# Dhia-naouali/dinov3-jax

Measured on NVIDIA H100. Metric: global_crops_per_sec, higher is better.
Workload: dtype bf16

## Files before the change

dinov3-jax_b200/csrc/attention.cu:

```cuda
#include "ptx.cuh"
#include <climits>
#include <cstdlib>
#include "d3_internal.h"

namespace d3 {

constexpr float LOG2E = 1.4426950408889634f;

__device__ long long* g_attn_dbg = nullptr;
__device__ __forceinline__ void dbg_mark(int slot) {
  if (g_attn_dbg && blockIdx.x == 0 && blockIdx.y == 0 && blockIdx.z == 0 && (threadIdx.x == 0 || threadIdx.x == 200))
    g_attn_dbg[slot * 2 + (threadIdx.x == 0 ? 0 : 1)] = clock64();
}

struct AttnShape {
  int G;
  int span;
  int n_crops;
  int N;
  int nkb;
  int D;
  int H;
  float scale;
  const float* sin_t;
  const float* cos_t;
  int prefix;
};

__device__ __forceinline__ uint32_t sw128_offset(int row, int col) {
  return (uint32_t)(row * 128 + ((((col >> 3) ^ (row & 7)) & 7) << 4) + (col & 7) * 2);
}

struct RowInfo { int g, klo, khi; bool ok; };
__device__ __forceinline__ RowInfo row_info(const AttnShape& sh, int c, int q) {
  RowInfo ri;
  ri.g = min(q / sh.N, sh.G - 1);
  ri.klo = ri.g * sh.N;
  ri.khi = ri.klo + sh.N;
  ri.ok = (q < sh.span) && (c * sh.G + ri.g < sh.n_crops);
  return ri;
}

template <int NI>
__device__ __forceinline__ void online_softmax(float (&s)[4 * NI], float (&o)[32], float (&m)[2], float (&l)[2],
                                               const RowInfo (&ri)[2], int k0, int c2, float cs) {
  const int kb0 = k0 + c2;
  const bool full = k0 >= max(ri[0].klo, ri[1].klo) && k0 + 8 * NI <= min(ri[0].khi, ri[1].khi);
  float mx[2] = {-3.0e38f, -3.0e38f};
#pragma unroll
  for (int i = 0; i < NI; ++i)
#pragma unroll
    for (int j = 0; j < 4; ++j) {
      const int hh = j >> 1, kk = kb0 + 8 * i + (j & 1);
      if (full || (kk >= ri[hh].klo && kk < ri[hh].khi)) mx[hh] = fmaxf(mx[hh], s[4 * i + j]);
    }
  float corr[2], ms[2];
#pragma unroll
  for (int hh = 0; hh < 2; ++hh) {
    mx[hh] = fmaxf(mx[hh], __shfl_xor_sync(0xffffffffu, mx[hh], 1));
    mx[hh] = fmaxf(mx[hh], __shfl_xor_sync(0xffffffffu, mx[hh], 2));
    const float mn = fmaxf(m[hh], mx[hh]);
    corr[hh] = ex2_approx((m[hh] - mn) * cs);
    m[hh] = mn;
    ms[hh] = mn * cs;
    l[hh] *= corr[hh];
  }
#pragma unroll
  for (int i = 0; i < NI; ++i)
#pragma unroll
    for (int j = 0; j < 4; ++j) {
      const int hh = j >> 1, kk = kb0 + 8 * i + (j & 1);
      const float p = (full || (kk >= ri[hh].klo && kk < ri[hh].khi)) ? ex2_approx(fmaf(s[4 * i + j], cs, -ms[hh])) : 0.f;
      s[4 * i + j] = p;
      l[hh] += p;
      if (i < 8) o[4 * i + j] *= corr[hh];
    }
}

__device__ __forceinline__ void store_o_lse(const float (&o)[32], float (&l)[2], const float (&m)[2], const RowInfo (&ri)[2],
                                            const AttnShape& sh, int c, int h, int row_base, int wq0, int r_in, int c2,
                                            __nv_bfloat16* O, float* LSE) {
#pragma unroll
  for (int hh = 0; hh < 2; ++hh) {
    l[hh] += __shfl_xor_sync(0xffffffffu, l[hh], 1);
    l[hh] += __shfl_xor_sync(0xffffffffu, l[hh], 2);
    const int q = wq0 + r_in + 8 * hh;
    if (!ri[hh].ok) continue;
    const float inv = 1.f / l[hh];
    __nv_bfloat16* dst = O + (size_t)(row_base + q) * sh.D + h * 64 + c2;
#pragma unroll
    for (int i = 0; i < 8; ++i)
      *reinterpret_cast<uint32_t*>(dst + 8 * i) = pack_bf16(o[4 * i + 2 * hh] * inv, o[4 * i + 2 * hh + 1] * inv);
    if (LSE && c2 == 0)
      LSE[((size_t)(c * sh.G + ri[hh].g) * sh.H + h) * sh.N + (q - ri[hh].klo)] = m[hh] * sh.scale + logf(l[hh]);
  }
}

__global__ void __launch_bounds__(256)
attn_fwd_kernel(const __grid_constant__ CUtensorMap tmQ, const __grid_constant__ CUtensorMap tmKV,
                __nv_bfloat16* __restrict__ O, float* __restrict__ LSE, const AttnShape sh) {
  extern __shared__ uint8_t smem_raw[];
  uint8_t* smem = reinterpret_cast<uint8_t*>((reinterpret_cast<uintptr_t>(smem_raw) + 1023) & ~uintptr_t(1023));
  uint8_t* sQ = smem;
  uint8_t* sK = smem + 16384;
  uint8_t* sV = sK + sh.nkb * 8192;
  uint64_t* bar = reinterpret_cast<uint64_t*>(sV + sh.nkb * 8192);

  const int wg = threadIdx.x >> 7, t = threadIdx.x & 127;
  const int qt = blockIdx.x, h = blockIdx.y, c = blockIdx.z;
  const int q0 = qt * 128;
  const int row_base = c * sh.span;
  dbg_mark(0);
  if (threadIdx.x == 0) {
    tma_prefetch_desc(&tmQ);
    tma_prefetch_desc(&tmKV);
    mbar_init(bar, 1);
    fence_mbar_init();
  }
  __syncthreads();
  if (threadIdx.x < 32 && elect_one()) {
    mbar_expect_tx(bar, 16384 + 2 * sh.nkb * 8192);
    tma_load_2d(&tmQ, bar, sQ, h * 64, row_base + q0);
    for (int b = 0; b < sh.nkb; ++b) {
      tma_load_2d(&tmKV, bar, sK + b * 8192, sh.D + h * 64, row_base + b * 64);
      tma_load_2d(&tmKV, bar, sV + b * 8192, 2 * sh.D + h * 64, row_base + b * 64);
    }
  }
  const int wq0 = q0 + wg * 64;
  if (wq0 >= sh.span) return;
  mbar_wait(bar, 0);

  const int r_in = 16 * (t >> 5) + ((t & 31) >> 2), c2 = 2 * (t & 3);
  RowInfo ri[2];
  ri[0] = row_info(sh, c, wq0 + r_in);
  ri[1] = row_info(sh, c, wq0 + r_in + 8);
  const int b_lo = (min(wq0 / sh.N, sh.G - 1) * sh.N) >> 6;
  const int b_hi = min(sh.nkb, ((min(min(wq0 + 63, sh.span - 1) / sh.N, sh.G - 1) + 1) * sh.N + 63) >> 6);
  const float cs = sh.scale * LOG2E;
  float m[2] = {-3.0e38f, -3.0e38f}, l[2] = {0.f, 0.f};
  float o[32];
#pragma unroll
  for (int i = 0; i < 32; ++i) o[i] = 0.f;
  const uint64_t qd = gmma_desc_sw128(smem_u32(sQ + wg * 8192), 16, 1024);

#pragma unroll 1
  for (int b = b_lo; b < b_hi; ++b) {
    float s[32];
    const uint64_t kd = gmma_desc_sw128(smem_u32(sK + b * 8192), 16, 1024);
    fence_regs(o);
    wgmma_fence();
#pragma unroll
    for (int k = 0; k < 4; ++k) wgmma_m64n64k16_ss<0, 0>(s, qd + 2 * k, kd + 2 * k, k > 0 ? 1u : 0u);
    wgmma_commit();
    wgmma_wait<0>();
    fence_regs(s);
    online_softmax<8>(s, o, m, l, ri, b * 64, c2, cs);
    uint32_t a[4][4];
#pragma unroll
    for (int kk = 0; kk < 4; ++kk)
#pragma unroll
      for (int e = 0; e < 4; ++e) a[kk][e] = pack_bf16(s[8 * kk + 2 * e], s[8 * kk + 2 * e + 1]);
    const uint64_t vd = gmma_desc_sw128(smem_u32(sV + b * 8192), 8192, 1024);
    fence_regs(o);
    wgmma_fence();
#pragma unroll
    for (int kk = 0; kk < 4; ++kk) wgmma_m64n64k16_rs<1>(o, a[kk], vd + 128 * kk, 1u);
    wgmma_commit();
    wgmma_wait<0>();
    fence_regs(o);
  }
  store_o_lse(o, l, m, ri, sh, c, h, row_base, wq0, r_in, c2, O, LSE);
  dbg_mark(1);
}

constexpr int FWD_STAGES = 4, DKDV_STAGES = 3, DQ_STAGES = 4;
constexpr int RING_THREADS = 384;

__global__ void __launch_bounds__(RING_THREADS, 1)
attn_fwd_stream_kernel(const __grid_constant__ CUtensorMap tmQKV, __nv_bfloat16* __restrict__ O, float* __restrict__ LSE,
                       const AttnShape sh) {
  extern __shared__ uint8_t smem_raw[];
  uint8_t* smem = reinterpret_cast<uint8_t*>((reinterpret_cast<uintptr_t>(smem_raw) + 1023) & ~uintptr_t(1023));
  uint8_t* sQ = smem;
  uint8_t* ring = smem + 16384;
  uint64_t* full = reinterpret_cast<uint64_t*>(ring + FWD_STAGES * 32768);
  uint64_t* empty = full + FWD_STAGES;
  uint64_t* bar_q = empty + FWD_STAGES;

  const int wg = threadIdx.x >> 7, t = threadIdx.x & 127;
  const int qt = blockIdx.x, h = blockIdx.y, c = blockIdx.z;
  const int q0 = qt * 128, row_base = c * sh.N, nkb = (sh.N + 127) >> 7;
  const int n_wg = (q0 + 64 < sh.N) ? 2 : 1;
  if (threadIdx.x == 0) {
    tma_prefetch_desc(&tmQKV);
    for (int st = 0; st < FWD_STAGES; ++st) {
      mbar_init(full + st, 1);
      mbar_init(empty + st, 4 * n_wg);
    }
    mbar_init(bar_q, 1);
    fence_mbar_init();
  }
  __syncthreads();
  if (wg == 2) {
    setmaxnreg_dec<40>();
    if (threadIdx.x < 288 && elect_one()) {
      mbar_expect_tx(bar_q, 16384);
      tma_load_2d(&tmQKV, bar_q, sQ, h * 64, row_base + q0);
      for (int b = 0; b < nkb; ++b) {
        const int st = b % FWD_STAGES, u = b / FWD_STAGES;
        if (u > 0) mbar_wait(empty + st, (u - 1) & 1);
        mbar_expect_tx(full + st, 32768);
        tma_load_2d(&tmQKV, full + st, ring + st * 32768, sh.D + h * 64, row_base + b * 128);
        tma_load_2d(&tmQKV, full + st, ring + st * 32768 + 16384, 2 * sh.D + h * 64, row_base + b * 128);
      }
    }
    return;
  }
  setmaxnreg_inc<232>();
  const int wq0 = q0 + wg * 64;
  if (wq0 >= sh.N) return;
  mbar_wait(bar_q, 0);

  const int r_in = 16 * (t >> 5) + ((t & 31) >> 2), c2 = 2 * (t & 3);
  RowInfo ri[2];
  ri[0] = row_info(sh, c, wq0 + r_in);
  ri[1] = row_info(sh, c, wq0 + r_in + 8);
  const float cs = sh.scale * LOG2E;
  float m[2] = {-3.0e38f, -3.0e38f}, l[2] = {0.f, 0.f};
  float o[32];
#pragma unroll
  for (int i = 0; i < 32; ++i) o[i] = 0.f;
  const uint64_t qd = gmma_desc_sw128(smem_u32(sQ + wg * 8192), 16, 1024);

#pragma unroll 1
  for (int b = 0; b < nkb; ++b) {
    const int st = b % FWD_STAGES;
    uint8_t* sK = ring + st * 32768;
    mbar_wait(full + st, (b / FWD_STAGES) & 1);
    float s[64];
    const uint64_t kd = gmma_desc_sw128(smem_u32(sK), 16, 1024);
    fence_regs(o);
    wgmma_fence();
#pragma unroll
    for (int k = 0; k < 4; ++k) wgmma_m64n128k16_ss<0, 0>(s, qd + 2 * k, kd + 2 * k, k > 0 ? 1u : 0u);
    wgmma_commit();
    wgmma_wait<0>();
    fence_regs(s);
    online_softmax<16>(s, o, m, l, ri, b * 128, c2, cs);
    uint32_t a[8][4];
#pragma unroll
    for (int kk = 0; kk < 8; ++kk)
#pragma unroll
      for (int e = 0; e < 4; ++e) a[kk][e] = pack_bf16(s[8 * kk + 2 * e], s[8 * kk + 2 * e + 1]);
    const uint64_t vd = gmma_desc_sw128(smem_u32(sK + 16384), 8192, 1024);
    fence_regs(o);
    wgmma_fence();
#pragma unroll
    for (int kk = 0; kk < 8; ++kk) wgmma_m64n64k16_rs<1>(o, a[kk], vd + 128 * kk, 1u);
    wgmma_commit();
    wgmma_wait<0>();
    fence_regs(o);
    if (lane_id() == 0) mbar_arrive(empty + st);
  }
  store_o_lse(o, l, m, ri, sh, c, h, row_base, wq0, r_in, c2, O, LSE);
}

__global__ void attn_delta_kernel(const __nv_bfloat16* __restrict__ O, const __nv_bfloat16* __restrict__ dO,
                                  float* __restrict__ delta, long T, int N, int D, int H) {
  const long g = blockIdx.x * (long)blockDim.x + threadIdx.x;
  const int per_row = D >> 3;
  const bool ok = g < T * per_row;
  float s = 0.f;
  long row = 0;
  int c8 = 0;
  if (ok) {
    row = g / per_row;
    c8 = (int)(g % per_row);
    const uint4 a = *reinterpret_cast<const uint4*>(O + row * D + c8 * 8);
    const uint4 b = *reinterpret_cast<const uint4*>(dO + row * D + c8 * 8);
    const float2 a0 = unpack_bf16(a.x), a1 = unpack_bf16(a.y), a2 = unpack_bf16(a.z), a3 = unpack_bf16(a.w);
    const float2 b0 = unpack_bf16(b.x), b1 = unpack_bf16(b.y), b2 = unpack_bf16(b.z), b3 = unpack_bf16(b.w);
    s = a0.x * b0.x + a0.y * b0.y + a1.x * b1.x + a1.y * b1.y + a2.x * b2.x + a2.y * b2.y + a3.x * b3.x + a3.y * b3.y;
  }
  s += __shfl_xor_sync(0xffffffffu, s, 4);
  s += __shfl_xor_sync(0xffffffffu, s, 2);
  s += __shfl_xor_sync(0xffffffffu, s, 1);
  if (ok && (c8 & 7) == 0) delta[((row / N) * H + (c8 >> 3)) * N + (row % N)] = s;
}

__device__ __forceinline__ void store_grad_rows(float (&a)[32], const AttnShape& sh, int c, int row_base, int tile_row0,
                                                int r_in, int c2, int h, int third, bool rope, __nv_bfloat16* dQKV) {
#pragma unroll
  for (int hh = 0; hh < 2; ++hh) {
    const int row = tile_row0 + r_in + 8 * hh;
    const RowInfo ri = row_info(sh, c, row);
    if (!ri.ok) continue;
    const int tok = row - ri.klo;
    float v[16];
#pragma unroll
    for (int i = 0; i < 8; ++i) { v[2 * i] = a[4 * i + 2 * hh]; v[2 * i + 1] = a[4 * i + 2 * hh + 1]; }
    if (rope && sh.sin_t && tok >= sh.prefix) {
      const float* sn = sh.sin_t + (size_t)(tok - sh.prefix) * 64;
      const float* cn = sh.cos_t + (size_t)(tok - sh.prefix) * 64;
#pragma unroll
      for (int i = 0; i < 4; ++i)
#pragma unroll
        for (int j = 0; j < 2; ++j) {
          const int d = 8 * i + c2 + j;
          const float lo = v[2 * i + j], hi = v[2 * (i + 4) + j];
          v[2 * i + j] = lo * cn[d] + hi * sn[d];
          v[2 * (i + 4) + j] = hi * cn[d] - lo * sn[d];
        }
    }
    __nv_bfloat16* dst = dQKV + (size_t)(row_base + row) * (3 * sh.D) + third * sh.D + h * 64 + c2;
#pragma unroll
    for (int i = 0; i < 8; ++i) *reinterpret_cast<uint32_t*>(dst + 8 * i) = pack_bf16(v[2 * i], v[2 * i + 1]);
  }
}

__device__ __forceinline__ void p_ds_tile(const AttnShape& sh, const float* __restrict__ LSE, const float* __restrict__ Delta,
                                          int c, int h, int q0, int kt, const uint8_t* sQw, const uint8_t* sDOw,
                                          const uint8_t* sK, const uint8_t* sV, int r_in, int c2, float (&s)[64],
                                          float (&dp)[64]) {
  const float cs = sh.scale * LOG2E;
  const uint64_t qd = gmma_desc_sw128(smem_u32(sQw), 16, 1024);
  const uint64_t dod = gmma_desc_sw128(smem_u32(sDOw), 16, 1024);
  const uint64_t kd = gmma_desc_sw128(smem_u32(sK), 16, 1024);
  const uint64_t vd = gmma_desc_sw128(smem_u32(sV), 16, 1024);
  wgmma_fence();
#pragma unroll
  for (int k = 0; k < 4; ++k) {
    wgmma_m64n128k16_ss<0, 0>(s, qd + 2 * k, kd + 2 * k, k > 0 ? 1u : 0u);
    wgmma_m64n128k16_ss<0, 0>(dp, dod + 2 * k, vd + 2 * k, k > 0 ? 1u : 0u);
  }
  wgmma_commit();
  wgmma_wait<0>();
  fence_regs(s);
  fence_regs(dp);
#pragma unroll
  for (int hh = 0; hh < 2; ++hh) {
    const int q = q0 + r_in + 8 * hh;
    const RowInfo ri = row_info(sh, c, q);
    const size_t stat = ((size_t)(c * sh.G + ri.g) * sh.H + h) * sh.N + (ri.ok ? q - ri.klo : 0);
    const float lse2 = ri.ok ? LSE[stat] * LOG2E : 0.f;
    const float dl = ri.ok ? Delta[stat] : 0.f;
    const int lo = ri.ok ? ri.klo - kt * 128 : 0, hi = ri.ok ? ri.khi - kt * 128 : 0;
#pragma unroll
    for (int i = 0; i < 16; ++i)
#pragma unroll
      for (int j = 0; j < 2; ++j) {
        const int e = 4 * i + 2 * hh + j, col = 8 * i + c2 + j;
        const bool ok = col >= lo && col < hi;
        const float p = ok ? ex2_approx(fmaf(s[e], cs, -lse2)) : 0.f;
        dp[e] = ok ? (p * sh.scale) * (dp[e] - dl) : 0.f;
        s[e] = p;
      }
  }
}

__device__ __forceinline__ void stash_p_ds(const float (&s)[64], const float (&dp)[64], uint8_t* sP, uint8_t* sDS, int row,
                                           int c2) {
#pragma unroll
  for (int hh = 0; hh < 2; ++hh) {
#pragma unroll
    for (int i = 0; i < 16; ++i) {
      const uint32_t off = (i >> 3) * 16384 + sw128_offset(row + 8 * hh, (8 * i + c2) & 63);
      *reinterpret_cast<uint32_t*>(sP + off) = pack_bf16(s[4 * i + 2 * hh], s[4 * i + 2 * hh + 1]);
      *reinterpret_cast<uint32_t*>(sDS + off) = pack_bf16(dp[4 * i + 2 * hh], dp[4 * i + 2 * hh + 1]);
    }
  }
}

__device__ __forceinline__ void dkdv_mma(float (&dk)[32], float (&dv)[32], const uint8_t* sP, const uint8_t* sDS,
                                         const uint8_t* sDOt, const uint8_t* sQt, int wg) {
  const uint64_t pd = gmma_desc_sw128(smem_u32(sP + wg * 16384), 16384, 1024);
  const uint64_t sd = gmma_desc_sw128(smem_u32(sDS + wg * 16384), 16384, 1024);
  const uint64_t dod = gmma_desc_sw128(smem_u32(sDOt), 8192, 1024);
  const uint64_t qd = gmma_desc_sw128(smem_u32(sQt), 8192, 1024);
  fence_regs(dk);
  fence_regs(dv);
  wgmma_fence();
#pragma unroll
  for (int k = 0; k < 8; ++k) {
    wgmma_m64n64k16_ss<1, 1>(dv, pd + 128 * k, dod + 128 * k, 1u);
    wgmma_m64n64k16_ss<1, 1>(dk, sd + 128 * k, qd + 128 * k, 1u);
  }
  wgmma_commit();
  wgmma_wait<0>();
  fence_regs(dk);
  fence_regs(dv);
}

__device__ __forceinline__ void dq_mma(float (&dq)[32], const float (&dp)[64], const uint8_t* sK) {
  uint32_t a[8][4];
#pragma unroll
  for (int kk = 0; kk < 8; ++kk)
#pragma unroll
    for (int e = 0; e < 4; ++e) a[kk][e] = pack_bf16(dp[8 * kk + 2 * e], dp[8 * kk + 2 * e + 1]);
  const uint64_t kd = gmma_desc_sw128(smem_u32(sK), 8192, 1024);
  fence_regs(dq);
  wgmma_fence();
#pragma unroll
  for (int kk = 0; kk < 8; ++kk) wgmma_m64n64k16_rs<1>(dq, a[kk], kd + 128 * kk, 1u);
  wgmma_commit();
  wgmma_wait<0>();
  fence_regs(dq);
}

__global__ void __launch_bounds__(256)
attn_bwd_kernel(const __grid_constant__ CUtensorMap tmQKV, const __grid_constant__ CUtensorMap tmDO,
                const float* __restrict__ LSE, const float* __restrict__ Delta, __nv_bfloat16* __restrict__ dQKV,
                const AttnShape sh) {
  extern __shared__ uint8_t smem_raw[];
  uint8_t* smem = reinterpret_cast<uint8_t*>((reinterpret_cast<uintptr_t>(smem_raw) + 1023) & ~uintptr_t(1023));
  const int nQ = (sh.span + 127) / 128, nK = nQ;
  uint8_t* sQ = smem;
  uint8_t* sDO = sQ + nQ * 16384;
  uint8_t* sK = sDO + nQ * 16384;
  uint8_t* sV = sK + 16384;
  uint8_t* sP = sV + 16384;
  uint8_t* sDS = sP + 32768;
  uint64_t* bars = reinterpret_cast<uint64_t*>(sDS + 32768);
  uint64_t* bar_q = bars;
  uint64_t* bar_kv = bars + 1;

  const int wg = threadIdx.x >> 7, t = threadIdx.x & 127;
  const int r_in = 16 * (t >> 5) + ((t & 31) >> 2), c2 = 2 * (t & 3);
  const int h = blockIdx.x, c = blockIdx.y;
  const int row_base = c * sh.span;
  dbg_mark(0);
  if (threadIdx.x == 0) {
    tma_prefetch_desc(&tmQKV);
    tma_prefetch_desc(&tmDO);
    mbar_init(bar_q, 1);
    mbar_init(bar_kv, 1);
    fence_mbar_init();
  }
  __syncthreads();
  if (threadIdx.x < 32 && elect_one()) {
    mbar_expect_tx(bar_q, nQ * 2 * 16384);
    for (int qt = 0; qt < nQ; ++qt) {
      tma_load_2d(&tmQKV, bar_q, sQ + qt * 16384, h * 64, row_base + qt * 128);
      tma_load_2d(&tmDO, bar_q, sDO + qt * 16384, h * 64, row_base + qt * 128);
    }
  }
  uint32_t kv_phase = 0;
  int kv_loaded = -1;
  auto load_kv = [&](int kt) {
    if (kv_loaded == kt) return;
    __syncthreads();
    if (threadIdx.x < 32 && elect_one()) {
      mbar_expect_tx(bar_kv, 2 * 16384);
      tma_load_2d(&tmQKV, bar_kv, sK, sh.D + h * 64, row_base + kt * 128);
      tma_load_2d(&tmQKV, bar_kv, sV, 2 * sh.D + h * 64, row_base + kt * 128);
    }
    mbar_wait(bar_kv, kv_phase);
    kv_phase ^= 1;
    kv_loaded = kt;
  };
  auto p_ds = [&](int qt, int kt, float (&s)[64], float (&dp)[64]) {
    p_ds_tile(sh, LSE, Delta, c, h, qt * 128 + wg * 64, kt, sQ + qt * 16384 + wg * 8192, sDO + qt * 16384 + wg * 8192,
              sK, sV, r_in, c2, s, dp);
  };

  mbar_wait(bar_q, 0);
#pragma unroll 1
  for (int kt = 0; kt < nK; ++kt) {
    load_kv(kt);
    float dk[32], dv[32];
#pragma unroll
    for (int i = 0; i < 32; ++i) { dk[i] = 0.f; dv[i] = 0.f; }
#pragma unroll 1
    for (int qt = 0; qt < nQ; ++qt) {
      float s[64], dp[64];
      p_ds(qt, kt, s, dp);
      stash_p_ds(s, dp, sP, sDS, wg * 64 + r_in, c2);
      fence_proxy_async_smem();
      __syncthreads();
      dkdv_mma(dk, dv, sP, sDS, sDO + qt * 16384, sQ + qt * 16384, wg);
      __syncthreads();
    }
    store_grad_rows(dk, sh, c, row_base, kt * 128 + wg * 64, r_in, c2, h, 1, true, dQKV);
    store_grad_rows(dv, sh, c, row_base, kt * 128 + wg * 64, r_in, c2, h, 2, false, dQKV);
  }
#pragma unroll 1
  for (int qt = 0; qt < nQ; ++qt) {
    float dq[32];
#pragma unroll
    for (int i = 0; i < 32; ++i) dq[i] = 0.f;
#pragma unroll 1
    for (int j = 0; j < nK; ++j) {
      const int kt = (qt & 1) ? j : nK - 1 - j;
      load_kv(kt);
      float s[64], dp[64];
      p_ds(qt, kt, s, dp);
      dq_mma(dq, dp, sK);
    }
    store_grad_rows(dq, sh, c, row_base, qt * 128 + wg * 64, r_in, c2, h, 0, true, dQKV);
  }
  dbg_mark(1);
}

__global__ void __launch_bounds__(RING_THREADS, 1)
attn_bwd_dkdv_kernel(const __grid_constant__ CUtensorMap tmQKV, const __grid_constant__ CUtensorMap tmDO,
                     const float* __restrict__ LSE, const float* __restrict__ Delta, __nv_bfloat16* __restrict__ dQKV,
                     const AttnShape sh) {
  extern __shared__ uint8_t smem_raw[];
  uint8_t* smem = reinterpret_cast<uint8_t*>((reinterpret_cast<uintptr_t>(smem_raw) + 1023) & ~uintptr_t(1023));
  uint8_t* sK = smem;
  uint8_t* sV = sK + 16384;
  uint8_t* sP = sV + 16384;
  uint8_t* sDS = sP + 32768;
  uint8_t* ring = sDS + 32768;
  uint64_t* full = reinterpret_cast<uint64_t*>(ring + DKDV_STAGES * 32768);
  uint64_t* empty = full + DKDV_STAGES;
  uint64_t* bar_kv = empty + DKDV_STAGES;

  const int wg = threadIdx.x >> 7, t = threadIdx.x & 127;
  const int r_in = 16 * (t >> 5) + ((t & 31) >> 2), c2 = 2 * (t & 3);
  const int kt = blockIdx.x, h = blockIdx.y, c = blockIdx.z;
  const int row_base = c * sh.N, nq = (sh.N + 127) >> 7;
  if (threadIdx.x == 0) {
    tma_prefetch_desc(&tmQKV);
    tma_prefetch_desc(&tmDO);
    for (int st = 0; st < DKDV_STAGES; ++st) {
      mbar_init(full + st, 1);
      mbar_init(empty + st, 8);
    }
    mbar_init(bar_kv, 1);
    fence_mbar_init();
  }
  __syncthreads();
  if (wg == 2) {
    setmaxnreg_dec<40>();
    if (threadIdx.x < 288 && elect_one()) {
      mbar_expect_tx(bar_kv, 32768);
      tma_load_2d(&tmQKV, bar_kv, sK, sh.D + h * 64, row_base + kt * 128);
      tma_load_2d(&tmQKV, bar_kv, sV, 2 * sh.D + h * 64, row_base + kt * 128);
      for (int qt = 0; qt < nq; ++qt) {
        const int st = qt % DKDV_STAGES, u = qt / DKDV_STAGES;
        if (u > 0) mbar_wait(empty + st, (u - 1) & 1);
        mbar_expect_tx(full + st, 32768);
        tma_load_2d(&tmQKV, full + st, ring + st * 32768, h * 64, row_base + qt * 128);
        tma_load_2d(&tmDO, full + st, ring + st * 32768 + 16384, h * 64, row_base + qt * 128);
      }
    }
    return;
  }
  setmaxnreg_inc<232>();
  mbar_wait(bar_kv, 0);
  float dk[32], dv[32];
#pragma unroll
  for (int i = 0; i < 32; ++i) { dk[i] = 0.f; dv[i] = 0.f; }
#pragma unroll 1
  for (int qt = 0; qt < nq; ++qt) {
    const int st = qt % DKDV_STAGES;
    const uint8_t* sQt = ring + st * 32768;
    const uint8_t* sDOt = sQt + 16384;
    mbar_wait(full + st, (qt / DKDV_STAGES) & 1);
    float s[64], dp[64];
    p_ds_tile(sh, LSE, Delta, c, h, qt * 128 + wg * 64, kt, sQt + wg * 8192, sDOt + wg * 8192, sK, sV, r_in, c2, s, dp);
    stash_p_ds(s, dp, sP, sDS, wg * 64 + r_in, c2);
    fence_proxy_async_smem();
    named_bar_sync(1, 256);
    dkdv_mma(dk, dv, sP, sDS, sDOt, sQt, wg);
    if (lane_id() == 0) mbar_arrive(empty + st);
    named_bar_sync(1, 256);
  }
  store_grad_rows(dk, sh, c, row_base, kt * 128 + wg * 64, r_in, c2, h, 1, true, dQKV);
  store_grad_rows(dv, sh, c, row_base, kt * 128 + wg * 64, r_in, c2, h, 2, false, dQKV);
}

__global__ void __launch_bounds__(RING_THREADS, 1)
attn_bwd_dq_kernel(const __grid_constant__ CUtensorMap tmQKV, const __grid_constant__ CUtensorMap tmDO,
                   const float* __restrict__ LSE, const float* __restrict__ Delta, __nv_bfloat16* __restrict__ dQKV,
                   const AttnShape sh) {
  extern __shared__ uint8_t smem_raw[];
  uint8_t* smem = reinterpret_cast<uint8_t*>((reinterpret_cast<uintptr_t>(smem_raw) + 1023) & ~uintptr_t(1023));
  uint8_t* sQ = smem;
  uint8_t* sDO = sQ + 16384;
  uint8_t* ring = sDO + 16384;
  uint64_t* full = reinterpret_cast<uint64_t*>(ring + DQ_STAGES * 32768);
  uint64_t* empty = full + DQ_STAGES;
  uint64_t* bar_q = empty + DQ_STAGES;

  const int wg = threadIdx.x >> 7, t = threadIdx.x & 127;
  const int r_in = 16 * (t >> 5) + ((t & 31) >> 2), c2 = 2 * (t & 3);
  const int qt = blockIdx.x, h = blockIdx.y, c = blockIdx.z;
  const int q0 = qt * 128, row_base = c * sh.N, nk = (sh.N + 127) >> 7;
  const int n_wg = (q0 + 64 < sh.N) ? 2 : 1;
  if (threadIdx.x == 0) {
    tma_prefetch_desc(&tmQKV);
    tma_prefetch_desc(&tmDO);
    for (int st = 0; st < DQ_STAGES; ++st) {
      mbar_init(full + st, 1);
      mbar_init(empty + st, 4 * n_wg);
    }
    mbar_init(bar_q, 1);
    fence_mbar_init();
  }
  __syncthreads();
  if (wg == 2) {
    setmaxnreg_dec<40>();
    if (threadIdx.x < 288 && elect_one()) {
      mbar_expect_tx(bar_q, 32768);
      tma_load_2d(&tmQKV, bar_q, sQ, h * 64, row_base + q0);
      tma_load_2d(&tmDO, bar_q, sDO, h * 64, row_base + q0);
      for (int kt = 0; kt < nk; ++kt) {
        const int st = kt % DQ_STAGES, u = kt / DQ_STAGES;
        if (u > 0) mbar_wait(empty + st, (u - 1) & 1);
        mbar_expect_tx(full + st, 32768);
        tma_load_2d(&tmQKV, full + st, ring + st * 32768, sh.D + h * 64, row_base + kt * 128);
        tma_load_2d(&tmQKV, full + st, ring + st * 32768 + 16384, 2 * sh.D + h * 64, row_base + kt * 128);
      }
    }
    return;
  }
  setmaxnreg_inc<232>();
  const int wq0 = q0 + wg * 64;
  if (wq0 >= sh.N) return;
  mbar_wait(bar_q, 0);
  float dq[32];
#pragma unroll
  for (int i = 0; i < 32; ++i) dq[i] = 0.f;
#pragma unroll 1
  for (int kt = 0; kt < nk; ++kt) {
    const int st = kt % DQ_STAGES;
    const uint8_t* sK = ring + st * 32768;
    mbar_wait(full + st, (kt / DQ_STAGES) & 1);
    float s[64], dp[64];
    p_ds_tile(sh, LSE, Delta, c, h, wq0, kt, sQ + wg * 8192, sDO + wg * 8192, sK, sK + 16384, r_in, c2, s, dp);
    dq_mma(dq, dp, sK);
    if (lane_id() == 0) mbar_arrive(empty + st);
  }
  store_grad_rows(dq, sh, c, row_base, wq0, r_in, c2, h, 0, true, dQKV);
}

static int make_map(CUtensorMap* map, const void* ptr, long rows, int cols, int ld, int box_rows) {
  cuuint64_t dims[2] = {(cuuint64_t)cols, (cuuint64_t)rows};
  cuuint64_t strides[1] = {(cuuint64_t)ld * 2};
  cuuint32_t box[2] = {64, (cuuint32_t)box_rows};
  cuuint32_t estr[2] = {1, 1};
  return encode_tensor_map_2d_bf16(map, ptr, dims, strides, box, estr);
}

constexpr int ATTN_MAX_TOKENS = 32768;
constexpr int ATTN_FWD_RESIDENT_SPAN = 448;
constexpr int ATTN_BWD_RESIDENT_N = 384;

static int attn_shape(AttnShape* s, int n_crops, int N, int D, int H) {
  if (D != H * 64) return set_error(D3_ERR_ARG, "attention: head_dim must be 64");
  if (N <= 0 || n_crops <= 0) return set_error(D3_ERR_ARG, "attention: empty problem");
  if (N > ATTN_MAX_TOKENS) return set_error(D3_ERR_ARG, "attention: N > 32768 tokens per crop");
  if ((long)n_crops * N > INT_MAX) return set_error(D3_ERR_ARG, "attention: n_crops * N must be below 2^31 token rows");
  s->N = N; s->D = D; s->H = H; s->scale = 0.125f; s->n_crops = n_crops;
  s->sin_t = nullptr; s->cos_t = nullptr; s->prefix = 0;
  s->G = (N <= 64) ? (128 / N) : 1;
  if (s->G > n_crops) s->G = n_crops;
  s->span = s->G * N;
  s->nkb = (s->span + 63) / 64;
  return D3_OK;
}

static int stream_grid(const AttnShape& s, dim3* grid) {
  if (s.H > 65535 || s.n_crops > 65535) return set_error(D3_ERR_ARG, "attention: H and n_crops must be <= 65535 for long crops");
  *grid = dim3((s.N + 127) / 128, s.H, s.n_crops);
  return D3_OK;
}

}

using namespace d3;

extern "C" {

int d3_debug_attn_trace(long long* buf ) {
  cudaError_t e = cudaMemcpyToSymbol(g_attn_dbg, &buf, sizeof(buf));
  return e == cudaSuccess ? D3_OK : set_error(D3_ERR_CUDA, cudaGetErrorString(e));
}

int d3_attn_fwd(const void* qkv, void* o, float* lse, int n_crops, int N, int D, int H, void* stream) {
  AttnShape s;
  int rc = attn_shape(&s, n_crops, N, D, H);
  if (rc) return rc;
  const long T = (long)n_crops * N;
  if (s.span > ATTN_FWD_RESIDENT_SPAN) {
    dim3 grid;
    if ((rc = stream_grid(s, &grid))) return rc;
    CUtensorMap tqkv;
    if ((rc = make_map(&tqkv, qkv, T, 3 * D, 3 * D, 128))) return rc;
    const int smem = 16384 + FWD_STAGES * 32768 + (2 * FWD_STAGES + 1) * 8 + 1024;
    static bool cfg_stream = false;
    if (!cfg_stream) {
      cudaFuncSetAttribute(attn_fwd_stream_kernel, cudaFuncAttributeMaxDynamicSharedMemorySize, smem);
      cfg_stream = true;
    }
    attn_fwd_stream_kernel<<<grid, RING_THREADS, smem, reinterpret_cast<cudaStream_t>(stream)>>>(tqkv, (__nv_bfloat16*)o,
                                                                                                 lse, s);
    D3_CHECK_LAUNCH();
    return D3_OK;
  }
  CUtensorMap tq, tkv;
  if ((rc = make_map(&tq, qkv, T, 3 * D, 3 * D, 128))) return rc;
  if ((rc = make_map(&tkv, qkv, T, 3 * D, 3 * D, 64))) return rc;
  const int smem = 16384 + 2 * s.nkb * 8192 + 64 + 1024;
  static bool cfg = false;
  if (!cfg) { cudaFuncSetAttribute(attn_fwd_kernel, cudaFuncAttributeMaxDynamicSharedMemorySize, 200 * 1024); cfg = true; }
  dim3 grid((s.span + 127) / 128, H, (n_crops + s.G - 1) / s.G);
  attn_fwd_kernel<<<grid, 256, smem, reinterpret_cast<cudaStream_t>(stream)>>>(tq, tkv, (__nv_bfloat16*)o, lse, s);
  D3_CHECK_LAUNCH();
  return D3_OK;
}

int d3_attn_bwd(const void* qkv, const void* o, const void* d_o, const float* lse, float* delta_scratch, void* dqkv,
                int n_crops, int N, int D, int H, const float* rope_sin, const float* rope_cos, int rope_prefix,
                void* stream) {
  AttnShape s;
  int rc = attn_shape(&s, n_crops, N, D, H);
  if (rc) return rc;
  if ((rope_sin == nullptr) != (rope_cos == nullptr)) return set_error(D3_ERR_ARG, "d3_attn_bwd: sin/cos tables");
  if (!delta_scratch) return set_error(D3_ERR_ARG, "d3_attn_bwd: delta scratch buffer");
  const bool streamed = N > ATTN_BWD_RESIDENT_N;
  dim3 sgrid;
  if (streamed && (rc = stream_grid(s, &sgrid))) return rc;
  s.sin_t = rope_sin; s.cos_t = rope_cos; s.prefix = rope_prefix;
  const long T = (long)n_crops * N;
  cudaStream_t st = reinterpret_cast<cudaStream_t>(stream);
  const long threads = T * (D / 8);
  attn_delta_kernel<<<(int)((threads + 255) / 256), 256, 0, st>>>((const __nv_bfloat16*)o, (const __nv_bfloat16*)d_o,
                                                                delta_scratch, T, N, D, H);
  D3_CHECK_LAUNCH();
  CUtensorMap tqkv, tdo;
  if ((rc = make_map(&tqkv, qkv, T, 3 * D, 3 * D, 128))) return rc;
  if ((rc = make_map(&tdo, d_o, T, D, D, 128))) return rc;
  if (streamed) {
    const int smem_kv = 16384 * 2 + 32768 * 2 + DKDV_STAGES * 32768 + (2 * DKDV_STAGES + 1) * 8 + 1024;
    const int smem_q = 16384 * 2 + DQ_STAGES * 32768 + (2 * DQ_STAGES + 1) * 8 + 1024;
    static bool cfg_stream = false;
    if (!cfg_stream) {
      cudaFuncSetAttribute(attn_bwd_dkdv_kernel, cudaFuncAttributeMaxDynamicSharedMemorySize, smem_kv);
      cudaFuncSetAttribute(attn_bwd_dq_kernel, cudaFuncAttributeMaxDynamicSharedMemorySize, smem_q);
      cfg_stream = true;
    }
    attn_bwd_dkdv_kernel<<<sgrid, RING_THREADS, smem_kv, st>>>(tqkv, tdo, lse, delta_scratch, (__nv_bfloat16*)dqkv, s);
    D3_CHECK_LAUNCH();
    attn_bwd_dq_kernel<<<sgrid, RING_THREADS, smem_q, st>>>(tqkv, tdo, lse, delta_scratch, (__nv_bfloat16*)dqkv, s);
    D3_CHECK_LAUNCH();
    return D3_OK;
  }
  static bool cfg = false;
  if (!cfg) { cudaFuncSetAttribute(attn_bwd_kernel, cudaFuncAttributeMaxDynamicSharedMemorySize, 226 * 1024); cfg = true; }
  const int nq = (s.span + 127) / 128;
  const int smem = 2 * nq * 16384 + 32768 + 65536 + 64 + 1024;
  dim3 grid(H, (n_crops + s.G - 1) / s.G);
  attn_bwd_kernel<<<grid, 256, smem, st>>>(tqkv, tdo, lse, delta_scratch, (__nv_bfloat16*)dqkv, s);
  D3_CHECK_LAUNCH();
  return D3_OK;
}

}
```

Baseline: 473.5.

## Fuse dQ into resident attention backward, computing S^T and dP^T once per tile pair

Replaces the resident backward kernel, which recomputed P and dS in a separate dQ pass, with a fused kernel. For each K/V and Q tile pair it computes the transposed scores and dP once, feeds them as register fragments into the dK/dV wgmma, stashes dS in shared memory and immediately accumulates dQ. When there are two tiles, a partial dQ is kept in shared memory. The change also adds per-tile mbarriers so loads overlap compute, preloads LSE and Delta into shared memory, and moves the resident/streamed threshold to span-based at 256. In exchange the synchronisation is more complex, the two-tile special cases are hand-coded, and crops with N between 257 and 384 are now routed to the streamed path.

Measured after the change: 490.1, median of 6. +3.5%, better.

```diff
diff --git a/dinov3-jax_b200/csrc/attention.cu b/dinov3-jax_b200/csrc/attention.cu
--- a/dinov3-jax_b200/csrc/attention.cu
+++ b/dinov3-jax_b200/csrc/attention.cu
@@ -407,22 +407,39 @@
   fence_regs(dq);
 }
 
-__global__ void __launch_bounds__(256)
-attn_bwd_kernel(const __grid_constant__ CUtensorMap tmQKV, const __grid_constant__ CUtensorMap tmDO,
-                const float* __restrict__ LSE, const float* __restrict__ Delta, __nv_bfloat16* __restrict__ dQKV,
-                const AttnShape sh) {
-  extern __shared__ uint8_t smem_raw[];
-  uint8_t* smem = reinterpret_cast<uint8_t*>((reinterpret_cast<uintptr_t>(smem_raw) + 1023) & ~uintptr_t(1023));
-  const int nQ = (sh.span + 127) / 128, nK = nQ;
-  uint8_t* sQ = smem;
-  uint8_t* sDO = sQ + nQ * 16384;
-  uint8_t* sK = sDO + nQ * 16384;
-  uint8_t* sV = sK + 16384;
-  uint8_t* sP = sV + 16384;
-  uint8_t* sDS = sP + 32768;
-  uint64_t* bars = reinterpret_cast<uint64_t*>(sDS + 32768);
-  uint64_t* bar_q = bars;
-  uint64_t* bar_kv = bars + 1;
+
+__host__ __device__ constexpr int bwd_fused_smem(int n_t) {
+  return n_t * 32768 * 2 + 32768 + (n_t > 1 ? 2 * 32768 : 0) + n_t * 128 * 8 + 2 * n_t * 8;
+}
+
+__device__ __forceinline__ uint64_t desc_here(const void* p, uint32_t lbo, uint32_t sbo) {
+  uint32_t a;
+  asm volatile("mov.b32 %0, %1;" : "=r"(a) : "r"(smem_u32(p)));
+  return gmma_desc_sw128(a, lbo, sbo);
+}
+
+__device__ __forceinline__ void fence_frag(uint32_t (&a)[4][4]) {
+#pragma unroll
+  for (int i = 0; i < 4; ++i)
+#pragma unroll
+    for (int e = 0; e < 4; ++e) asm volatile("" : "+r"(a[i][e])::"memory");
+}
+
+__global__ void __launch_bounds__(256, 1)
+attn_bwd_fused_kernel(const __grid_constant__ CUtensorMap tmQKV, const __grid_constant__ CUtensorMap tmDO,
+                      const float* __restrict__ LSE, const float* __restrict__ Delta, __nv_bfloat16* __restrict__ dQKV,
+                      const AttnShape sh) {
+  extern __shared__ __align__(1024) uint8_t smem_al[];
+  const int nT = (sh.span + 127) / 128;
+  uint8_t* sKV = smem_al;
+  uint8_t* sQDO = sKV + nT * 32768;
+  uint8_t* sDS = sQDO + nT * 32768;
+  uint8_t* sDS0 = sDS + 32768;
+  float* sDQ = reinterpret_cast<float*>(sDS0 + 32768);
+  float* sLSE = reinterpret_cast<float*>(sDS + (nT > 1 ? 3 * 32768 : 32768));
+  float* sDel = sLSE + nT * 128;
+  uint64_t* bar_kv = reinterpret_cast<uint64_t*>(sDel + nT * 128);
+  uint64_t* bar_q = bar_kv + nT;
 
   const int wg = threadIdx.x >> 7, t = threadIdx.x & 127;
   const int r_in = 16 * (t >> 5) + ((t & 31) >> 2), c2 = 2 * (t & 3);
@@ -432,71 +449,167 @@
   if (threadIdx.x == 0) {
     tma_prefetch_desc(&tmQKV);
     tma_prefetch_desc(&tmDO);
-    mbar_init(bar_q, 1);
-    mbar_init(bar_kv, 1);
+    for (int i = 0; i < 2 * nT; ++i) mbar_init(bar_kv + i, 1);
     fence_mbar_init();
   }
   __syncthreads();
   if (threadIdx.x < 32 && elect_one()) {
-    mbar_expect_tx(bar_q, nQ * 2 * 16384);
-    for (int qt = 0; qt < nQ; ++qt) {
-      tma_load_2d(&tmQKV, bar_q, sQ + qt * 16384, h * 64, row_base + qt * 128);
-      tma_load_2d(&tmDO, bar_q, sDO + qt * 16384, h * 64, row_base + qt * 128);
-    }
-  }
-  uint32_t kv_phase = 0;
-  int kv_loaded = -1;
-  auto load_kv = [&](int kt) {
-    if (kv_loaded == kt) return;
-    __syncthreads();
-    if (threadIdx.x < 32 && elect_one()) {
-      mbar_expect_tx(bar_kv, 2 * 16384);
-      tma_load_2d(&tmQKV, bar_kv, sK, sh.D + h * 64, row_base + kt * 128);
-      tma_load_2d(&tmQKV, bar_kv, sV, 2 * sh.D + h * 64, row_base + kt * 128);
-    }
-    mbar_wait(bar_kv, kv_phase);
-    kv_phase ^= 1;
-    kv_loaded = kt;
-  };
-  auto p_ds = [&](int qt, int kt, float (&s)[64], float (&dp)[64]) {
-    p_ds_tile(sh, LSE, Delta, c, h, qt * 128 + wg * 64, kt, sQ + qt * 16384 + wg * 8192, sDO + qt * 16384 + wg * 8192,
-              sK, sV, r_in, c2, s, dp);
-  };
-
-  mbar_wait(bar_q, 0);
+    for (int i = 0; i < nT; ++i) {
+      mbar_expect_tx(bar_kv + i, 32768);
+      tma_load_2d(&tmQKV, bar_kv + i, sKV + i * 32768, sh.D + h * 64, row_base + i * 128);
+      tma_load_2d(&tmQKV, bar_kv + i, sKV + i * 32768 + 16384, 2 * sh.D + h * 64, row_base + i * 128);
+      mbar_expect_tx(bar_q + i, 32768);
+      tma_load_2d(&tmQKV, bar_q + i, sQDO + i * 32768, h * 64, row_base + i * 128);
+      tma_load_2d(&tmDO, bar_q + i, sQDO + i * 32768 + 16384, h * 64, row_base + i * 128);
+    }
+  }
+  for (int q = threadIdx.x; q < nT * 128; q += 256) {
+    const RowInfo ri = row_info(sh, c, q);
+    const size_t stat = ((size_t)(c * sh.G + ri.g) * sh.H + h) * sh.N + (q - ri.klo);
+    sLSE[q] = ri.ok ? LSE[stat] * LOG2E : 0.f;
+    sDel[q] = ri.ok ? Delta[stat] : 0.f;
+  }
+  __syncthreads();
+
+  const float cs = sh.scale * LOG2E;
+  int pair = 0;
 #pragma unroll 1
-  for (int kt = 0; kt < nK; ++kt) {
-    load_kv(kt);
+  for (int kt = 0; kt < nT; ++kt) {
+    mbar_wait(bar_kv + kt, 0);
+    const uint8_t* sK = sKV + kt * 32768;
+    const uint8_t* sV = sK + 16384;
+    int lo[2], hi[2];
+#pragma unroll
+    for (int hh = 0; hh < 2; ++hh) {
+      const RowInfo ri = row_info(sh, c, kt * 128 + wg * 64 + r_in + 8 * hh);
+      lo[hh] = ri.ok ? ri.klo : 0;
+      hi[hh] = ri.ok ? ri.khi : 0;
+    }
     float dk[32], dv[32];
-#pragma unroll
-    for (int i = 0; i < 32; ++i) { dk[i] = 0.f; dv[i] = 0.f; }
 #pragma unroll 1
-    for (int qt = 0; qt < nQ; ++qt) {
-      float s[64], dp[64];
-      p_ds(qt, kt, s, dp);
-      stash_p_ds(s, dp, sP, sDS, wg * 64 + r_in, c2);
+    for (int qt = 0; qt < nT; ++qt, ++pair) {
+      mbar_wait(bar_q + qt, 0);
+      const uint8_t* sQt = sQDO + qt * 32768;
+      const uint8_t* sDOt = sQt + 16384;
+      const bool defer = nT == 2 && kt == 0 && qt == 0;
+      uint8_t* stash = defer ? sDS0 : sDS;
+      uint32_t pa[2][4][4], da[2][4][4];
+#pragma unroll
+      for (int hf = 0; hf < 2; ++hf) {
+        float s[32], dp[32];
+        {
+          const uint64_t kd = desc_here(sK + wg * 8192, 16, 1024);
+          const uint64_t vd = desc_here(sV + wg * 8192, 16, 1024);
+          const uint64_t qd = desc_here(sQt + hf * 8192, 16, 1024);
+          const uint64_t dod = desc_here(sDOt + hf * 8192, 16, 1024);
+          wgmma_fence();
+#pragma unroll
+          for (int k = 0; k < 4; ++k) {
+            wgmma_m64n64k16_ss<0, 0>(s, kd + 2 * k, qd + 2 * k, k > 0 ? 1u : 0u);
+            wgmma_m64n64k16_ss<0, 0>(dp, vd + 2 * k, dod + 2 * k, k > 0 ? 1u : 0u);
+          }
+          wgmma_commit();
+          wgmma_wait<0>();
+          fence_regs(s);
+          fence_regs(dp);
+          if (hf == 1) { fence_frag(pa[0]); fence_frag(da[0]); }
+        }
+        const float* lse2 = sLSE + qt * 128 + hf * 64;
+        const float* del = sDel + qt * 128 + hf * 64;
+#pragma unroll
+        for (int i = 0; i < 8; ++i) {
+          const int col = 8 * i + c2;
+          const float2 l2 = *reinterpret_cast<const float2*>(lse2 + col);
+          const float2 dl = *reinterpret_cast<const float2*>(del + col);
+          const int q = qt * 128 + hf * 64 + col;
+          float pv[4], dv4[4];
+#pragma unroll
+          for (int j = 0; j < 4; ++j) {
+            const int hh = j >> 1, qq = q + (j & 1);
+            const bool ok = qq >= lo[hh] && qq < hi[hh];
+            const float p = ok ? ex2_approx(fmaf(s[4 * i + j], cs, -((j & 1) ? l2.y : l2.x))) : 0.f;
+            dv4[j] = ok ? (p * sh.scale) * (dp[4 * i + j] - ((j & 1) ? dl.y : dl.x)) : 0.f;
+            pv[j] = p;
+          }
+          pa[hf][i >> 1][2 * (i & 1)] = pack_bf16(pv[0], pv[1]);
+          pa[hf][i >> 1][2 * (i & 1) + 1] = pack_bf16(pv[2], pv[3]);
+          da[hf][i >> 1][2 * (i & 1)] = pack_bf16(dv4[0], dv4[1]);
+          da[hf][i >> 1][2 * (i & 1) + 1] = pack_bf16(dv4[2], dv4[3]);
+        }
+        if (hf == 0 && pair > 1) named_bar_sync(1, 256);
+#pragma unroll
+        for (int hh = 0; hh < 2; ++hh)
+#pragma unroll
+          for (int i = 0; i < 8; ++i) {
+            const uint32_t off = hf * 16384 + sw128_offset(wg * 64 + r_in + 8 * hh, 8 * i + c2);
+            *reinterpret_cast<uint32_t*>(stash + off) = da[hf][i >> 1][2 * (i & 1) + hh];
+          }
+        {
+          const uint64_t dod = desc_here(sDOt, 8192, 1024);
+          const uint64_t qd = desc_here(sQt, 8192, 1024);
+          const uint32_t acc_on = (qt > 0 || hf > 0) ? 1u : 0u;
+          if (acc_on) { fence_regs(dk); fence_regs(dv); }
+          wgmma_fence();
+#pragma unroll
+          for (int kk = 0; kk < 4; ++kk) {
+            const int ks = 4 * hf + kk;
+            wgmma_m64n64k16_rs<1>(dv, pa[hf][kk], dod + 128 * ks, (acc_on || kk > 0) ? 1u : 0u);
+            wgmma_m64n64k16_rs<1>(dk, da[hf][kk], qd + 128 * ks, (acc_on || kk > 0) ? 1u : 0u);
+          }
+          wgmma_commit();
+        }
+      }
       fence_proxy_async_smem();
-      __syncthreads();
-      dkdv_mma(dk, dv, sP, sDS, sDO + qt * 16384, sQ + qt * 16384, wg);
-      __syncthreads();
+      if (defer) {
+        wgmma_wait<0>();
+        fence_regs(dk);
+        fence_regs(dv);
+        fence_frag(pa[1]);
+        fence_frag(da[1]);
+        continue;
+      }
+      named_bar_sync(2, 256);
+      const bool from_partial = nT == 2 && kt == 1 && qt == 1;
+      float dq[32];
+      float4* part = reinterpret_cast<float4*>(sDQ) + wg * 8 * 128 + t;
+      if (from_partial) {
+#pragma unroll
+        for (int j = 0; j < 8; ++j) {
+          const float4 v = part[j * 128];
+          dq[4 * j] = v.x; dq[4 * j + 1] = v.y; dq[4 * j + 2] = v.z; dq[4 * j + 3] = v.w;
+        }
+      }
+      {
+        const uint64_t sd = desc_here(sDS + wg * 16384, 16384, 1024);
+        const uint64_t kbd = desc_here(sK, 8192, 1024);
+        fence_regs(dq);
+        wgmma_fence();
+#pragma unroll
+        for (int kk = 0; kk < 8; ++kk)
+          wgmma_m64n64k16_ss<1, 1>(dq, sd + 128 * kk, kbd + 128 * kk, (from_partial || kk > 0) ? 1u : 0u);
+        if (nT == 2 && kt == 1 && qt == 0) {
+          const uint64_t sd0 = desc_here(sDS0 + wg * 16384, 16384, 1024);
+          const uint64_t k0d = desc_here(sKV, 8192, 1024);
+#pragma unroll
+          for (int kk = 0; kk < 8; ++kk) wgmma_m64n64k16_ss<1, 1>(dq, sd0 + 128 * kk, k0d + 128 * kk, 1u);
+        }
+        wgmma_commit();
+        wgmma_wait<0>();
+        fence_regs(dq);
+        fence_regs(dk);
+        fence_regs(dv);
+        fence_frag(pa[1]);
+        fence_frag(da[1]);
+      }
+      if (nT == 2 && kt == 0) {
+#pragma unroll
+        for (int j = 0; j < 8; ++j) part[j * 128] = make_float4(dq[4 * j], dq[4 * j + 1], dq[4 * j + 2], dq[4 * j + 3]);
+      } else {
+        store_grad_rows(dq, sh, c, row_base, qt * 128 + wg * 64, r_in, c2, h, 0, true, dQKV);
+      }
     }
     store_grad_rows(dk, sh, c, row_base, kt * 128 + wg * 64, r_in, c2, h, 1, true, dQKV);
     store_grad_rows(dv, sh, c, row_base, kt * 128 + wg * 64, r_in, c2, h, 2, false, dQKV);
-  }
-#pragma unroll 1
-  for (int qt = 0; qt < nQ; ++qt) {
-    float dq[32];
-#pragma unroll
-    for (int i = 0; i < 32; ++i) dq[i] = 0.f;
-#pragma unroll 1
-    for (int j = 0; j < nK; ++j) {
-      const int kt = (qt & 1) ? j : nK - 1 - j;
-      load_kv(kt);
-      float s[64], dp[64];
-      p_ds(qt, kt, s, dp);
-      dq_mma(dq, dp, sK);
-    }
-    store_grad_rows(dq, sh, c, row_base, qt * 128 + wg * 64, r_in, c2, h, 0, true, dQKV);
   }
   dbg_mark(1);
 }
@@ -646,7 +759,7 @@
 
 constexpr int ATTN_MAX_TOKENS = 32768;
 constexpr int ATTN_FWD_RESIDENT_SPAN = 448;
-constexpr int ATTN_BWD_RESIDENT_N = 384;
+constexpr int ATTN_BWD_RESIDENT_SPAN = 256;
 
 static int attn_shape(AttnShape* s, int n_crops, int N, int D, int H) {
   if (D != H * 64) return set_error(D3_ERR_ARG, "attention: head_dim must be 64");
@@ -720,7 +833,7 @@
   if (rc) return rc;
   if ((rope_sin == nullptr) != (rope_cos == nullptr)) return set_error(D3_ERR_ARG, "d3_attn_bwd: sin/cos tables");
   if (!delta_scratch) return set_error(D3_ERR_ARG, "d3_attn_bwd: delta scratch buffer");
-  const bool streamed = N > ATTN_BWD_RESIDENT_N;
+  const bool streamed = s.span > ATTN_BWD_RESIDENT_SPAN;
   dim3 sgrid;
   if (streamed && (rc = stream_grid(s, &sgrid))) return rc;
   s.sin_t = rope_sin; s.cos_t = rope_cos; s.prefix = rope_prefix;
@@ -749,11 +862,13 @@
     return D3_OK;
   }
   static bool cfg = false;
-  if (!cfg) { cudaFuncSetAttribute(attn_bwd_kernel, cudaFuncAttributeMaxDynamicSharedMemorySize, 226 * 1024); cfg = true; }
-  const int nq = (s.span + 127) / 128;
-  const int smem = 2 * nq * 16384 + 32768 + 65536 + 64 + 1024;
+  if (!cfg) {
+    cudaFuncSetAttribute(attn_bwd_fused_kernel, cudaFuncAttributeMaxDynamicSharedMemorySize, bwd_fused_smem(2));
+    cfg = true;
+  }
   dim3 grid(H, (n_crops + s.G - 1) / s.G);
-  attn_bwd_kernel<<<grid, 256, smem, st>>>(tqkv, tdo, lse, delta_scratch, (__nv_bfloat16*)dqkv, s);
+  attn_bwd_fused_kernel<<<grid, 256, bwd_fused_smem((s.span + 127) / 128), st>>>(tqkv, tdo, lse, delta_scratch,
+                                                                                 (__nv_bfloat16*)dqkv, s);
   D3_CHECK_LAUNCH();
   return D3_OK;
 }
```
